# KwonGihyun/TweedieMix

Hardware: AMD Instinct MI355X
Metric: denoise steps/sec @ SDXL 1024^2 K=3 concepts (fusion phase); images/sec at 1/2/4/8 GPUs (higher is better)
Workload: dtype bf16

## Files before the change

### tweediemix_amd/csrc/conv_io.hip

```cpp
#include "common.h"

namespace {

struct PreMap { float w[16]; float b[4]; int on; };

template <int CIN>
__global__ void __launch_bounds__(256) conv_in_kernel(const float* __restrict__ x, const float* __restrict__ w,
                                                      const float* __restrict__ bias, bf16_t* __restrict__ y,
                                                      int B, int H, int W, int Cout, const PreMap pm) {
    extern __shared__ __attribute__((aligned(16))) float s_w[];
    constexpr int KK = 9 * CIN;
    const int tid = threadIdx.x, lane = tid & 63;
    const int q = __builtin_amdgcn_readfirstlane(tid >> 6);
    for (int i = tid; i < Cout * KK / 4; i += 256) ((float4*)s_w)[i] = ((const float4*)w)[i];
    __syncthreads();
    const int64_t npix = (int64_t)B * H * W;
    for (int64_t tile = blockIdx.x; tile * 64 < npix; tile += gridDim.x) {
    int64_t pix = tile * 64 + lane;
    const bool live = pix < npix;
    if (!live) pix = npix - 1;
    const int b = (int)(pix / ((int64_t)H * W)); const int rem = (int)(pix - (int64_t)b * H * W);
    const int oy = rem / W, ox = rem - oy * W;
    float patch[KK];
#pragma unroll
    for (int ky = 0; ky < 3; ++ky)
#pragma unroll
        for (int kx = 0; kx < 3; ++kx) {
            const int iy = oy + ky - 1, ix = ox + kx - 1;
            const bool ok = iy >= 0 && iy < H && ix >= 0 && ix < W;
            float v[CIN];
#pragma unroll
            for (int ci = 0; ci < CIN; ++ci) v[ci] = ok ? x[(((int64_t)b * CIN + ci) * H + iy) * W + ix] : 0.f;
            if (pm.on && CIN == 4) {
                float u[4];
#pragma unroll
                for (int co = 0; co < 4; ++co)
                    u[co] = ok ? pm.b[co] + pm.w[co * 4 + 0] * v[0] + pm.w[co * 4 + 1] * v[1] + pm.w[co * 4 + 2] * v[2] + pm.w[co * 4 + 3] * v[3] : 0.f;
#pragma unroll
                for (int co = 0; co < 4; ++co) v[co] = u[co];
            }
#pragma unroll
            for (int ci = 0; ci < CIN; ++ci) patch[(ky * 3 + kx) * CIN + ci] = v[ci];
        }
    const int cpq = Cout / 4;
    for (int c0 = q * cpq; c0 < (q + 1) * cpq; c0 += 8) {
        float o[8];
#pragma unroll 2
        for (int j = 0; j < 8; ++j) {
            const float* wr = s_w + (c0 + j) * KK;
            float a = bias ? bias[c0 + j] : 0.f;
#pragma unroll
            for (int k = 0; k < KK; ++k) a += patch[k] * wr[k];
            o[j] = a;
        }
        if (live) *(uint4*)(y + pix * Cout + c0) = pack8(o);
    }
    }
}

template <int CIN>
int launch_conv_in(unsigned nb, int smem, hipStream_t st, const float* x, const float* w, const float* bias, bf16_t* y, int B, int H, int W, int Cout, const PreMap& pm) {
    static int attr_smem = 0;
    if (smem > 64 * 1024 && smem > attr_smem) {
        hipError_t e = hipFuncSetAttribute((const void*)conv_in_kernel<CIN>, hipFuncAttributeMaxDynamicSharedMemorySize, smem);
        if (e != hipSuccess) TMIX_FAIL((int)e, "hipFuncSetAttribute: %s", hipGetErrorString(e));
        attr_smem = smem;
    }
    conv_in_kernel<CIN><<<nb, 256, smem, st>>>(x, w, bias, y, B, H, W, Cout, pm);
    TMIX_LAUNCH_CHECK();
    return TMIX_OK;
}

__global__ void __launch_bounds__(256) conv_out_kernel(const bf16_t* __restrict__ x, const bf16_t* __restrict__ w,
                                                       const float* __restrict__ bias, float* __restrict__ y,
                                                       int B, int H, int W, int Cin, int Cout) {
    const int lane = threadIdx.x & 63, fr = lane & 15, fg = lane >> 4;
    const int64_t npix = (int64_t)B * H * W;
    const int64_t pbase = ((int64_t)blockIdx.x * 4 + (threadIdx.x >> 6)) * 16;
    if (pbase >= npix) return;
    int64_t pix = pbase + fr; if (pix > npix - 1) pix = npix - 1;
    const int b = (int)(pix / ((int64_t)H * W)); const int rem = (int)(pix - (int64_t)b * H * W);
    const int oy = rem / W, ox = rem - oy * W;
    const int co = fr < Cout ? fr : Cout - 1;
    const bf16_t* wrow = w + (int64_t)co * 9 * Cin;
    f32x4 acc = {0.f, 0.f, 0.f, 0.f};
    const frag_ab zero = {0, 0, 0, 0, 0, 0, 0, 0};
    for (int tap = 0; tap < 9; ++tap) {
        const int ky = tap / 3, kx = tap - ky * 3;
        const int iy = oy + ky - 1, ix = ox + kx - 1;
        const bool ok = iy >= 0 && iy < H && ix >= 0 && ix < W;
        const bf16_t* src = x + (((int64_t)b * H + (ok ? iy : 0)) * W + (ok ? ix : 0)) * Cin;
        for (int c = 0; c < Cin; c += 32) {
            frag_ab a = *(const frag_ab*)(src + c + fg * 8);
            if (!ok) a = zero;
            const frag_ab wf = *(const frag_ab*)(wrow + tap * Cin + c + fg * 8);
            acc = __builtin_amdgcn_mfma_f32_16x16x32_bf16(a, wf, acc, 0, 0, 0);
        }
    }
    if (fr < Cout) {
        const float bv = bias ? bias[fr] : 0.f;
#pragma unroll
        for (int r = 0; r < 4; ++r) {
            const int64_t pp = pbase + fg * 4 + r;
            if (pp < npix) {
                const int bb = (int)(pp / ((int64_t)H * W)); const int64_t rr = pp - (int64_t)bb * H * W;
                y[((int64_t)bb * Cout + fr) * H * W + rr] = acc[r] + bv;
            }
        }
    }
}

}

extern "C" int tmix_conv_in(const float* x_nchw, const float* w_ohwi, const float* bias, void* y_nhwc,
                            int B, int Cin, int H, int W, int Cout, void* stream) {
    return tmix_conv_in_pre(x_nchw, w_ohwi, bias, y_nhwc, B, Cin, H, W, Cout, nullptr, nullptr, stream);
}

extern "C" int tmix_conv_in_pre(const float* x_nchw, const float* w_ohwi, const float* bias, void* y_nhwc,
                                int B, int Cin, int H, int W, int Cout, const float* pre_w, const float* pre_b, void* stream) {
    if (!x_nchw || !w_ohwi || !y_nhwc) TMIX_FAIL(TMIX_EINVAL, "conv_in: null pointer");
    if (B <= 0 || H <= 0 || W <= 0 || Cout <= 0) TMIX_FAIL(TMIX_ESHAPE, "conv_in: bad shape");
    if (!aligned16(y_nhwc)) TMIX_FAIL(TMIX_EALIGN, "conv_in: output must be 16-byte aligned");
    if (Cout % 32) TMIX_FAIL(TMIX_ESHAPE, "conv_in: Cout=%d must be a multiple of 32", Cout);
    if (Cin != 3 && Cin != 4 && Cin != 8) TMIX_FAIL(TMIX_ESHAPE, "conv_in: Cin=%d (3: RGB image, 4: image latent, 8: video latent + image-latent features)", Cin);
    if (Cin != 4 && pre_w) TMIX_FAIL(TMIX_EINVAL, "conv_in: the latent pre-map is defined for 4 channels");
    if ((Cout * 9 * Cin) % 4) TMIX_FAIL(TMIX_ESHAPE, "conv_in: Cout*9*Cin must be a multiple of 4");
    if (!aligned16(w_ohwi)) TMIX_FAIL(TMIX_EALIGN, "conv_in: weights must be 16-byte aligned");
    const int64_t npix = (int64_t)B * H * W;
    const int64_t ntiles = (npix + 63) / 64;
    const int smem = Cout * 9 * Cin * 4;
    const int per_cu = smem > 80 * 1024 ? 1 : (smem > 52 * 1024 ? 2 : 3);
    const unsigned nb = (unsigned)(ntiles < 256 * per_cu ? ntiles : 256 * per_cu);
    if (smem > 150 * 1024) TMIX_FAIL(TMIX_ESHAPE, "conv_in: Cout=%d too large for the LDS weight stage", Cout);
    PreMap pm = {};
    if (pre_w) {
        pm.on = 1;
        for (int i = 0; i < 16; ++i) pm.w[i] = pre_w[i];
        for (int i = 0; i < 4; ++i) pm.b[i] = pre_b ? pre_b[i] : 0.f;
    }
    hipStream_t st = (hipStream_t)stream;
    bf16_t* y = (bf16_t*)y_nhwc;
    switch (Cin) {
        case 8:  return launch_conv_in<8>(nb, smem, st, x_nchw, w_ohwi, bias, y, B, H, W, Cout, pm);
        case 3:  return launch_conv_in<3>(nb, smem, st, x_nchw, w_ohwi, bias, y, B, H, W, Cout, pm);
        default: return launch_conv_in<4>(nb, smem, st, x_nchw, w_ohwi, bias, y, B, H, W, Cout, pm);
    }
}

extern "C" int tmix_conv_out(const void* x_nhwc, const void* w_ohwi, const float* bias, float* y_nchw,
                             int B, int Cin, int H, int W, int Cout, void* stream) {
    if (!x_nhwc || !w_ohwi || !y_nchw) TMIX_FAIL(TMIX_EINVAL, "conv_out: null pointer");
    if (B <= 0 || H <= 0 || W <= 0 || Cout <= 0 || Cout > 16 || (Cin % 32)) TMIX_FAIL(TMIX_ESHAPE, "conv_out: Cin=%d (%%32) Cout=%d (<=16)", Cin, Cout);
    if (!aligned16(x_nhwc) || !aligned16(w_ohwi)) TMIX_FAIL(TMIX_EALIGN, "conv_out: pointers must be 16-byte aligned");
    const int64_t npix = (int64_t)B * H * W;
    const unsigned nb = (unsigned)((npix + 63) / 64);
    conv_out_kernel<<<nb, 256, 0, (hipStream_t)stream>>>((const bf16_t*)x_nhwc, (const bf16_t*)w_ohwi, bias, y_nchw, B, H, W, Cin, Cout);
    TMIX_LAUNCH_CHECK();
    return TMIX_OK;
}
```

Baseline: 32.43.

## Move conv_in to fp32 MFMA and tile conv_out through LDS halo staging

conv_in drops the per-thread scalar FMA loop over a 9*Cin patch. Weights are now laid out in LDS in MFMA fragment order, and the conv is computed with 16x16x4 fp32 MFMA instructions, with bias preloaded into LDS. conv_out changes from per-pixel global gathers for each tap to 8x16 spatial tiles: a halo of input channels is staged in LDS in 64-channel chunks, the next chunk is prefetched into registers, and the 9 tap weights are reused across two output rows per wave. This reduces redundant global reads and scalar ALU work, at the cost of more complex indexing, extra LDS traffic and barriers. Both conv_in and conv_out are small parts of the UNet step.

```diff
diff --git a/tweediemix_amd/csrc/conv_io.hip b/tweediemix_amd/csrc/conv_io.hip
--- a/tweediemix_amd/csrc/conv_io.hip
+++ b/tweediemix_amd/csrc/conv_io.hip
@@ -3,58 +3,72 @@
 namespace {
 
 struct PreMap { float w[16]; float b[4]; int on; };
+
+template <int CIN> struct ConvInGeom {
+    static constexpr int KK = 9 * CIN;
+    static constexpr int NS = (KK + 3) / 4;
+};
+inline int conv_in_steps(int Cin) { return (9 * Cin + 3) / 4; }
+inline int conv_in_lds_bytes(int Cin, int Cout) { return Cout * (conv_in_steps(Cin) * 16 + 4); }
 
 template <int CIN>
 __global__ void __launch_bounds__(256) conv_in_kernel(const float* __restrict__ x, const float* __restrict__ w,
                                                       const float* __restrict__ bias, bf16_t* __restrict__ y,
                                                       int B, int H, int W, int Cout, const PreMap pm) {
     extern __shared__ __attribute__((aligned(16))) float s_w[];
-    constexpr int KK = 9 * CIN;
-    const int tid = threadIdx.x, lane = tid & 63;
+    constexpr int KK = ConvInGeom<CIN>::KK, NS = ConvInGeom<CIN>::NS;
+    const int tid = threadIdx.x, lane = tid & 63, fr = lane & 15, fg = lane >> 4;
     const int q = __builtin_amdgcn_readfirstlane(tid >> 6);
-    for (int i = tid; i < Cout * KK / 4; i += 256) ((float4*)s_w)[i] = ((const float4*)w)[i];
+    const int nfrag = Cout * NS * 4;
+    for (int e = tid; e < nfrag; e += 256) {
+        const int l = e & 63, f = e >> 6;
+        const int s = f % NS, bh = f / NS;
+        const int i = l & 15, k = 4 * s + (l >> 4);
+        const int ch = (bh >> 1) * 32 + (i >> 2) * 8 + (bh & 1) * 4 + (i & 3);
+        s_w[e] = k < KK ? w[ch * KK + k] : 0.f;
+    }
+    float* s_b = s_w + nfrag;
+    for (int c = tid; c < Cout; c += 256) s_b[c] = bias ? bias[c] : 0.f;
     __syncthreads();
     const int64_t npix = (int64_t)B * H * W;
     for (int64_t tile = blockIdx.x; tile * 64 < npix; tile += gridDim.x) {
-    int64_t pix = tile * 64 + lane;
-    const bool live = pix < npix;
-    if (!live) pix = npix - 1;
-    const int b = (int)(pix / ((int64_t)H * W)); const int rem = (int)(pix - (int64_t)b * H * W);
-    const int oy = rem / W, ox = rem - oy * W;
-    float patch[KK];
-#pragma unroll
-    for (int ky = 0; ky < 3; ++ky)
-#pragma unroll
-        for (int kx = 0; kx < 3; ++kx) {
+        if (tile * 64 + q * 16 >= npix) continue;
+        int64_t pix = tile * 64 + q * 16 + fr;
+        const bool live = pix < npix;
+        if (!live) pix = npix - 1;
+        const int b = (int)(pix / ((int64_t)H * W)); const int rem = (int)(pix - (int64_t)b * H * W);
+        const int oy = rem / W, ox = rem - oy * W;
+        float xf[NS];
+#pragma unroll
+        for (int s = 0; s < NS; ++s) {
+            const int k = 4 * s + fg;
+            const int tap = k / CIN, ci = k - tap * CIN;
+            const int ky = tap / 3, kx = tap - ky * 3;
             const int iy = oy + ky - 1, ix = ox + kx - 1;
-            const bool ok = iy >= 0 && iy < H && ix >= 0 && ix < W;
-            float v[CIN];
-#pragma unroll
-            for (int ci = 0; ci < CIN; ++ci) v[ci] = ok ? x[(((int64_t)b * CIN + ci) * H + iy) * W + ix] : 0.f;
+            const bool ok = k < KK && iy >= 0 && iy < H && ix >= 0 && ix < W;
             if (pm.on && CIN == 4) {
-                float u[4];
+                float v[4], u[4];
+#pragma unroll
+                for (int c = 0; c < 4; ++c) v[c] = ok ? x[(((int64_t)b * CIN + c) * H + iy) * W + ix] : 0.f;
 #pragma unroll
                 for (int co = 0; co < 4; ++co)
                     u[co] = ok ? pm.b[co] + pm.w[co * 4 + 0] * v[0] + pm.w[co * 4 + 1] * v[1] + pm.w[co * 4 + 2] * v[2] + pm.w[co * 4 + 3] * v[3] : 0.f;
-#pragma unroll
-                for (int co = 0; co < 4; ++co) v[co] = u[co];
-            }
-#pragma unroll
-            for (int ci = 0; ci < CIN; ++ci) patch[(ky * 3 + kx) * CIN + ci] = v[ci];
-        }
-    const int cpq = Cout / 4;
-    for (int c0 = q * cpq; c0 < (q + 1) * cpq; c0 += 8) {
-        float o[8];
-#pragma unroll 2
-        for (int j = 0; j < 8; ++j) {
-            const float* wr = s_w + (c0 + j) * KK;
-            float a = bias ? bias[c0 + j] : 0.f;
-#pragma unroll
-            for (int k = 0; k < KK; ++k) a += patch[k] * wr[k];
-            o[j] = a;
-        }
-        if (live) *(uint4*)(y + pix * Cout + c0) = pack8(o);
-    }
+                xf[s] = fg == 0 ? u[0] : fg == 1 ? u[1] : fg == 2 ? u[2] : u[3];
+            } else {
+                xf[s] = ok ? x[(((int64_t)b * CIN + ci) * H + iy) * W + ix] : 0.f;
+            }
+        }
+        for (int g = 0; g < Cout / 32; ++g) {
+            const float* wa = s_w + g * 2 * NS * 64 + lane;
+            f32x4 a0 = *(const f32x4*)(s_b + g * 32 + fg * 8), a1 = *(const f32x4*)(s_b + g * 32 + fg * 8 + 4);
+#pragma unroll
+            for (int s = 0; s < NS; ++s) {
+                a0 = __builtin_amdgcn_mfma_f32_16x16x4f32(wa[s * 64], xf[s], a0, 0, 0, 0);
+                a1 = __builtin_amdgcn_mfma_f32_16x16x4f32(wa[(NS + s) * 64], xf[s], a1, 0, 0, 0);
+            }
+            const float o[8] = {a0[0], a0[1], a0[2], a0[3], a1[0], a1[1], a1[2], a1[3]};
+            if (live) *(uint4*)(y + pix * Cout + g * 32 + fg * 8) = pack8(o);
+        }
     }
 }
 
@@ -71,40 +85,87 @@
     return TMIX_OK;
 }
 
+constexpr int CONV_OUT_ROWS = 8, CONV_OUT_COLS = 16, CONV_OUT_CHUNK = 64;
+constexpr int CO_HALO_W = CONV_OUT_COLS + 2, CO_HALO_PIX = (CONV_OUT_ROWS + 2) * CO_HALO_W;
+constexpr int CO_PLANES = CONV_OUT_CHUNK / 8;
+constexpr int CO_PLANE_BYTES = (CO_HALO_PIX * 16 + 255) / 256 * 256;
+constexpr int CO_PIECES = CO_HALO_PIX * CO_PLANES;
+constexpr int CO_TRIPS = (CO_PIECES + 255) / 256;
+static_assert(CONV_OUT_ROWS == 8 && CONV_OUT_COLS == 16, "four waves x two rows of one 16-pixel MFMA tile");
+
 __global__ void __launch_bounds__(256) conv_out_kernel(const bf16_t* __restrict__ x, const bf16_t* __restrict__ w,
                                                        const float* __restrict__ bias, float* __restrict__ y,
-                                                       int B, int H, int W, int Cin, int Cout) {
-    const int lane = threadIdx.x & 63, fr = lane & 15, fg = lane >> 4;
-    const int64_t npix = (int64_t)B * H * W;
-    const int64_t pbase = ((int64_t)blockIdx.x * 4 + (threadIdx.x >> 6)) * 16;
-    if (pbase >= npix) return;
-    int64_t pix = pbase + fr; if (pix > npix - 1) pix = npix - 1;
-    const int b = (int)(pix / ((int64_t)H * W)); const int rem = (int)(pix - (int64_t)b * H * W);
-    const int oy = rem / W, ox = rem - oy * W;
+                                                       int B, int H, int W, int Cin, int Cout, int ntx, int nty) {
+    __shared__ __attribute__((aligned(256))) unsigned char s_a[CO_PLANES * CO_PLANE_BYTES];
+    const int tid = threadIdx.x, lane = tid & 63, fr = lane & 15, fg = lane >> 4;
+    const int q = __builtin_amdgcn_readfirstlane(tid >> 6);
+    int bid = blockIdx.x;
+    const int tx = bid % ntx; bid /= ntx;
+    const int ty = bid % nty, b = bid / nty;
+    const int y0 = ty * CONV_OUT_ROWS, x0 = tx * CONV_OUT_COLS;
+    int64_t src[CO_TRIPS]; int dst[CO_TRIPS];
+#pragma unroll
+    for (int t = 0; t < CO_TRIPS; ++t) {
+        const int it = tid + t * 256;
+        const int pl = it / CO_HALO_PIX, hp = it - pl * CO_HALO_PIX;
+        const int hy = hp / CO_HALO_W, hx = hp - hy * CO_HALO_W;
+        const int iy = y0 - 1 + hy, ix = x0 - 1 + hx;
+        const bool inside = it < CO_PIECES && iy >= 0 && iy < H && ix >= 0 && ix < W;
+        src[t] = inside ? (((int64_t)b * H + iy) * W + ix) * Cin + pl * 8 : -1;
+        dst[t] = it < CO_PIECES ? pl * CO_PLANE_BYTES + hp * 16 : -1;
+    }
+    uint4 piece[CO_TRIPS];
+    auto fetch = [&](int c0) {
+#pragma unroll
+        for (int t = 0; t < CO_TRIPS; ++t) {
+            const int pl = (tid + t * 256) / CO_HALO_PIX;
+            piece[t] = src[t] >= 0 && c0 + pl * 8 < Cin ? *(const uint4*)(x + src[t] + c0) : make_uint4(0u, 0u, 0u, 0u);
+        }
+    };
     const int co = fr < Cout ? fr : Cout - 1;
-    const bf16_t* wrow = w + (int64_t)co * 9 * Cin;
-    f32x4 acc = {0.f, 0.f, 0.f, 0.f};
+    const bf16_t* wrow = w + (int64_t)co * 9 * Cin + fg * 8;
+    const int a_off = fg * CO_PLANE_BYTES + (q * 2 * CO_HALO_W + fr) * 16;
     const frag_ab zero = {0, 0, 0, 0, 0, 0, 0, 0};
-    for (int tap = 0; tap < 9; ++tap) {
-        const int ky = tap / 3, kx = tap - ky * 3;
-        const int iy = oy + ky - 1, ix = ox + kx - 1;
-        const bool ok = iy >= 0 && iy < H && ix >= 0 && ix < W;
-        const bf16_t* src = x + (((int64_t)b * H + (ok ? iy : 0)) * W + (ok ? ix : 0)) * Cin;
-        for (int c = 0; c < Cin; c += 32) {
-            frag_ab a = *(const frag_ab*)(src + c + fg * 8);
-            if (!ok) a = zero;
-            const frag_ab wf = *(const frag_ab*)(wrow + tap * Cin + c + fg * 8);
-            acc = __builtin_amdgcn_mfma_f32_16x16x32_bf16(a, wf, acc, 0, 0, 0);
-        }
+    f32x4 acc[2] = {{0.f, 0.f, 0.f, 0.f}, {0.f, 0.f, 0.f, 0.f}};
+    fetch(0);
+    for (int c0 = 0; c0 < Cin; c0 += CONV_OUT_CHUNK) {
+        const int nks = Cin - c0 >= CONV_OUT_CHUNK ? 2 : 1;
+        frag_ab wf[9][2];
+#pragma unroll
+        for (int tap = 0; tap < 9; ++tap)
+#pragma unroll
+            for (int ks = 0; ks < 2; ++ks)
+                wf[tap][ks] = ks < nks ? *(const frag_ab*)(wrow + tap * Cin + c0 + ks * 32) : zero;
+#pragma unroll
+        for (int t = 0; t < CO_TRIPS; ++t)
+            if (dst[t] >= 0) *(uint4*)(s_a + dst[t]) = piece[t];
+        __syncthreads();
+        if (c0 + CONV_OUT_CHUNK < Cin) fetch(c0 + CONV_OUT_CHUNK);
+#pragma unroll
+        for (int tap = 0; tap < 9; ++tap) {
+            const int ky = tap / 3, kx = tap - ky * 3;
+#pragma unroll
+            for (int ks = 0; ks < 2; ++ks) {
+                if (ks < nks) {
+#pragma unroll
+                    for (int t = 0; t < 2; ++t) {
+                        const frag_ab a = *(const frag_ab*)(s_a + a_off + ks * 4 * CO_PLANE_BYTES + ((t + ky) * CO_HALO_W + kx) * 16);
+                        acc[t] = __builtin_amdgcn_mfma_f32_16x16x32_bf16(a, wf[tap][ks], acc[t], 0, 0, 0);
+                    }
+                }
+            }
+        }
+        __syncthreads();
     }
     if (fr < Cout) {
         const float bv = bias ? bias[fr] : 0.f;
 #pragma unroll
-        for (int r = 0; r < 4; ++r) {
-            const int64_t pp = pbase + fg * 4 + r;
-            if (pp < npix) {
-                const int bb = (int)(pp / ((int64_t)H * W)); const int64_t rr = pp - (int64_t)bb * H * W;
-                y[((int64_t)bb * Cout + fr) * H * W + rr] = acc[r] + bv;
+        for (int t = 0; t < 2; ++t) {
+            const int oy = y0 + q * 2 + t;
+#pragma unroll
+            for (int r = 0; r < 4; ++r) {
+                const int ox = x0 + fg * 4 + r;
+                if (oy < H && ox < W) y[(((int64_t)b * Cout + fr) * H + oy) * W + ox] = acc[t][r] + bv;
             }
         }
     }
@@ -129,10 +190,10 @@
     if (!aligned16(w_ohwi)) TMIX_FAIL(TMIX_EALIGN, "conv_in: weights must be 16-byte aligned");
     const int64_t npix = (int64_t)B * H * W;
     const int64_t ntiles = (npix + 63) / 64;
-    const int smem = Cout * 9 * Cin * 4;
+    if (Cout * 9 * Cin * 4 > 150 * 1024) TMIX_FAIL(TMIX_ESHAPE, "conv_in: Cout=%d too large for the LDS weight stage", Cout);
+    const int smem = conv_in_lds_bytes(Cin, Cout);
     const int per_cu = smem > 80 * 1024 ? 1 : (smem > 52 * 1024 ? 2 : 3);
     const unsigned nb = (unsigned)(ntiles < 256 * per_cu ? ntiles : 256 * per_cu);
-    if (smem > 150 * 1024) TMIX_FAIL(TMIX_ESHAPE, "conv_in: Cout=%d too large for the LDS weight stage", Cout);
     PreMap pm = {};
     if (pre_w) {
         pm.on = 1;
@@ -153,9 +214,9 @@
     if (!x_nhwc || !w_ohwi || !y_nchw) TMIX_FAIL(TMIX_EINVAL, "conv_out: null pointer");
     if (B <= 0 || H <= 0 || W <= 0 || Cout <= 0 || Cout > 16 || (Cin % 32)) TMIX_FAIL(TMIX_ESHAPE, "conv_out: Cin=%d (%%32) Cout=%d (<=16)", Cin, Cout);
     if (!aligned16(x_nhwc) || !aligned16(w_ohwi)) TMIX_FAIL(TMIX_EALIGN, "conv_out: pointers must be 16-byte aligned");
-    const int64_t npix = (int64_t)B * H * W;
-    const unsigned nb = (unsigned)((npix + 63) / 64);
-    conv_out_kernel<<<nb, 256, 0, (hipStream_t)stream>>>((const bf16_t*)x_nhwc, (const bf16_t*)w_ohwi, bias, y_nchw, B, H, W, Cin, Cout);
+    const int ntx = (W + CONV_OUT_COLS - 1) / CONV_OUT_COLS, nty = (H + CONV_OUT_ROWS - 1) / CONV_OUT_ROWS;
+    const unsigned nb = (unsigned)((int64_t)B * nty * ntx);
+    conv_out_kernel<<<nb, 256, 0, (hipStream_t)stream>>>((const bf16_t*)x_nhwc, (const bf16_t*)w_ohwi, bias, y_nchw, B, H, W, Cin, Cout, ntx, nty);
     TMIX_LAUNCH_CHECK();
     return TMIX_OK;
 }
```

After: 32.50, median of 6. No clear change (+0.2%).
